# asbschmidt/CUDASW4

Hardware: AMD Instinct MI355X
Metric: GCUPS (higher is better)
Workload: dtype f16x2; 1 GPU; peak: allqueries.fasta (20 queries, 41752 residues) vs pseudo DB 1000000 x 512, half2 kernel configuration, blosum62, gop -11 gex -1, top 10, C++ host driver; db_subjects=1000000, db_residues=512000000, queries=20, kernel=half2, queries_in_flight=1, tail_overlaps=10, numa_node_rank0=1, numa_bound=True, resident=True, residency=resident, cached_chars=512000000, parallelism=db-shard x1 (one DB sharded), one top-K gather per step + host merge

## Files before the change

### cudasw4_amd/csrc/sw_api.hip

```cpp
#include <hip/hip_runtime.h>
#include <hipcub/hipcub.hpp>

#include <algorithm>
#include <cstdio>
#include <cmath>
#include <cstdlib>
#include <cstring>
#include <ctime>
#include <string>
#include <vector>

#include "../../include/cudasw4_amd.h"
#include "../../include/cudasw4_amd_engine.h"
#include "../../include/cudasw4_amd_pssm.h"
#include "sw_internal.hpp"
#include "sw_launch.hpp"
#include "sw_pssm.hpp"
#include "sw_rows_pipeline.hpp"

namespace {

thread_local std::string g_last_error = "";

int fail(int code, const std::string& msg) {
// ... 175 lines not shown
    if (part_id < SW_NUM_LENGTH_PARTITIONS - 2) {
        if (!ctx->have_query) return 16;
        const int32_t limit4 = ctx->lanes4_max_q >= 0 ? ctx->lanes4_max_q : kind_packed(kind) ? SW_LANES4_MAX_QUERY_PACKED : SW_LANES4_MAX_QUERY_SCALAR;
        const int64_t batches4 = (int64_t)n / (64 * (kind_packed(kind) ? 2 : 1));
        const bool enough4 = ctx->lanes4_max_q >= 0 || batches4 >= (int64_t)SW_LANES4_MIN_BATCHES_PER_CU * std::max(1, ctx->num_cus);
        const int32_t lmax4 = ctx->lanes4_max_subject >= 0 ? ctx->lanes4_max_subject : SW_LANES4_MAX_SUBJECT;
        if (ctx->qlen <= 4 * swk::max_rows(kind, 4) && ctx->qlen <= limit4 && enough4 && max_subject_len <= lmax4) return 4;
        const bool fits8 = ctx->qlen <= 8 * swk::max_rows(kind, 8);
        const int32_t limit = ctx->lanes8_max_q >= 0 ? ctx->lanes8_max_q : kind_packed(kind) ? SW_LANES8_MAX_QUERY_PACKED : SW_LANES8_MAX_QUERY_SCALAR;
        if (fits8 && ctx->qlen <= limit) return 8;
        return 16;
    }
    const int64_t fills_gpu_twice = (int64_t)2 * std::max(1, ctx->num_cus) * 4 * 32;
    if (part_id == SW_NUM_LENGTH_PARTITIONS - 2) return n >= (ctx->long16_min >= 0 ? ctx->long16_min : 512) ? 16 : 64;
    return n >= fills_gpu_twice ? 16 : 64;
}


int ensure_profile(sw_ctx* ctx, int kind, int lanes, int frame, int shift, hipStream_t stream) {
    Profile& pr = ctx->profiles[kind][shape_index(lanes)][frame];
    if (pr.valid && pr.shift != shift) pr.valid = false;
    if (pr.valid) {
        SW_HIP(hipStreamWaitEvent(stream, pr.ready, 0));
        return SW_OK;
    }
    const swk::KindLaunch* kl = kind_launch(kind);
    const QueryPlan pl = plan_query(kind, ctx->qlen, lanes);
    const size_t bytes = kl->tile_bytes(pl.rows, lanes) * (size_t)pl.nstripes;
    if (bytes == 0) return fail(SW_ERR_INVALID, "no kernel compiled for this query plan");
    if (bytes > pr.capacity) {
        const size_t cap = std::max<size_t>(std::max(bytes, 2 * pr.capacity), size_t(2) << 20);
        if (pr.dev) SW_HIP(hipFree(pr.dev));
        pr.dev = nullptr;
        pr.capacity = 0;
        SW_HIP(hipMalloc(&pr.dev, cap));
        pr.capacity = cap;
    }
    if (ctx->pssm_mode) SW_HIP(kl->profile(pl.rows, lanes, nullptr, ctx->qlen, ctx->d_pssm, ctx->qlen, pl.nstripes, pr.dev, shift, frame == 2 ? 1 : 0, stream));
    else SW_HIP(kl->profile(pl.rows, lanes, ctx->d_query, ctx->qlen, ctx->d_matrix, ctx->dim, pl.nstripes, pr.dev, shift, frame == 2 ? 1 : 0, stream));
    pr.shift = shift;
    if (!pr.ready) SW_HIP(hipEventCreateWithFlags(&pr.ready, hipEventDisableTiming));
    SW_HIP(hipEventRecord(pr.ready, stream));
    pr.plan = pl;
    pr.valid = true;
    return SW_OK;
}

int32_t border_capacity(int32_t max_len, int lanes) {
    const int64_t steps = ((int64_t)max_len + lanes - 1 + 3) / 4 * 4;
    return (int32_t)((steps + 15) / 16 * 16 + 16);
}
size_t border_bytes_per_wg(int32_t lcap, int lanes) {
    if (lanes == 4) return 0;
    const size_t region = lanes == 16 ? swk::border_region_words<16>(lcap) : lanes == 8 ? swk::border_region_words<8>(lcap) : swk::border_region_words<64>(lcap);
    return (size_t)(swk::kThreads / lanes) * region * sizeof(uint32_t);
}

__global__ void max_length_kernel(const int32_t* lengths, const int32_t* positions, const int32_t* count_ptr, int32_t first_pos,
                                  int32_t n, int32_t* out) {
    const int32_t cnt = count_ptr ? min(*count_ptr, n) : n;
    int32_t m = 0;
    for (int32_t i = blockIdx.x * blockDim.x + threadIdx.x; i < cnt; i += gridDim.x * blockDim.x)
        m = max(m, lengths[positions ? positions[i] : first_pos + i]);
    if (m > 0) atomicMax(out, m);
}

struct StreamPlan { int slots = 0, cols = 0, room = 0, base = 0, jump = 0; };
StreamPlan stream_plan(const sw_ctx* ctx, int kind, int lanes, int a, const QueryPlan& pl, int32_t max_subject_len) {
    StreamPlan sp;
    if (!kind_packed(kind) || lanes != 16 || a < 0) return sp;
    const bool multi = pl.nstripes > 1;
    const int P = swk::frame_classes(true, pl.rows, lanes, multi);
    sp.base = kind == SW_KIND_F16X2 ? -2016 : 0;
    const int top = kind == SW_KIND_F16X2 ? 1024 : 12400;
    sp.jump = ctx->stream_jump > 0 ? ctx->stream_jump : (kind == SW_KIND_F16X2 ? 512 : 2048);
    sp.room = top - sp.base - a * (2 * lanes + 4 + P);
    sp.cols = a > 0 ? std::min(sp.room / a, ctx->stream_cols_max) : ctx->stream_cols_max;
    sp.slots = std::max(1, std::min(ctx->stream_slots, swk::kStreamMaxSlots));
    if (sp.room < 4 * lanes * a || sp.cols < 4 * lanes) sp.slots = 1;
    if (multi) {
        const int32_t limit = ctx->stream_multi_max_subject >= 0 ? ctx->stream_multi_max_subject : (kind == SW_KIND_F16X2 ? 320 : 192);
        if (max_subject_len > limit) sp.slots = 1;
        sp.cols = std::min(sp.cols, ctx->stream_multi_cols_max);
    }
    return sp;
}

bool offs_possible(const sw_ctx* ctx, int kind, int lanes, int32_t max_subject_len, int gop, int gex, int ovf_check, int64_t* K_out) {
    const int a = -gex;
    const int64_t room = kind == SW_KIND_F16X2 ? 1536 : kind == SW_KIND_I16X2 ? 12500 : (int64_t)1 << 22;
    int64_t K = 1 << 21;
    while (K >= 4 * lanes && (int64_t)a * (K + 3 * lanes + 16) > room) K >>= 1;
    if (kind == SW_KIND_I16X2) K = std::min<int64_t>(K, std::max<int64_t>(2048, 4 * lanes));
    if (!kind_packed(kind) && max_subject_len + 3 * lanes + 16 > K) K = 0;
    if (K_out) *K_out = K;
    return ctx->use_offs && K >= 4 * lanes && (!kind_packed(kind) || (ovf_check && a >= 0)) && gop - gex >= -1000;
}
int packed_fallback_kind(int kind) { return kind == SW_KIND_F16X2 ? SW_KIND_F32 : SW_KIND_I32; }

constexpr uint32_t kWorkZeroBlock = 64;
hipError_t take_work_slot(sw_ctx* ctx, hipStream_t stream, uint32_t** out) {
    uint32_t* w = ctx->d_work + 2 * (ctx->work_next++ % kWorkSlots);
    *out = w;
    if (ctx->work_zeroed > 0) { ctx->work_zeroed--; return hipSuccess; }
    return hipMemsetAsync(w, 0, 2 * sizeof(uint32_t), stream);
}

// ... 1347 lines not shown
```

### cudasw4_amd/csrc/sw_dp_kernel.hpp

```cpp
#pragma once

#include <hip/hip_runtime.h>
#include <stdint.h>

#include <type_traits>

#include "sw_pssm.hpp"

namespace swk {

typedef uint32_t u32;
typedef short s16x2 __attribute__((ext_vector_type(2)));
typedef unsigned short u16x2 __attribute__((ext_vector_type(2)));
typedef _Float16 f16x2 __attribute__((ext_vector_type(2)));

constexpr int kGroup = 16;
constexpr int kThreads = 256;
constexpr int kPadLetter = 20;
constexpr int kLetters = 21;

enum { F16X2 = 0, I16X2 = 1, I32 = 2, F32 = 3 };

constexpr int DPP_ROW_SHL1 = 0x101;
constexpr int DPP_ROW_SHR1 = 0x111;
// ... 325 lines not shown
#define SWK_WAVES4_MAX_R 22
#endif
#ifndef SWK_CLASSES_PACKED
#define SWK_CLASSES_PACKED 8
#endif
#ifndef SWK_CLASSES_PACKED_SMALL
#define SWK_CLASSES_PACKED_SMALL 4
#endif
#ifndef SWK_CLASSES_SCALAR
#define SWK_CLASSES_SCALAR 4
#endif
constexpr int frame_classes(bool packed, int R, int lanes, bool multi, bool uniform = false) {
    (void)lanes;
    const int want = packed ? ((R > SWK_WAVES3_MAX_R || (multi && R >= 25 && (uniform || R > SWK_WAVES3_MAX_R_MULTI))) ? SWK_CLASSES_PACKED : SWK_CLASSES_PACKED_SMALL)
                            : SWK_CLASSES_SCALAR;
    int P = want;
    while (P > 1 && 2 * P > R) P--;
    return P;
}

constexpr int kLookahead = 12;

template <int NW, int CHUNK_ROW_BYTES>
__device__ __forceinline__ void lds_read_chunk2(u32 (&da)[NW], u32 (&db)[NW], const unsigned char* pa, const unsigned char* pb, int c) {
    lds_read_chunk<NW, CHUNK_ROW_BYTES>(da, pa, c);
    lds_read_chunk<NW, CHUNK_ROW_BYTES>(db, pb, c);
    __builtin_amdgcn_sched_barrier(0);
}

template <int NW, int CHUNK_ROW_BYTES>
__device__ __forceinline__ void lds_read_words2(u32 (&da)[NW], u32 (&db)[NW], const unsigned char* pa, const unsigned char* pb) {
#pragma unroll
    for (int c = 0; c < Chunks<NW>::kCount; c++) lds_read_chunk2<NW, CHUNK_ROW_BYTES>(da, db, pa, pb, c);
}

template <int NW, int CHUNK_ROW_BYTES>
__device__ __forceinline__ void lds_read_chunk1(u32 (&da)[NW], const unsigned char* pa, int c) {
    lds_read_chunk<NW, CHUNK_ROW_BYTES>(da, pa, c);
    __builtin_amdgcn_sched_barrier(0);
}

template <int KIND, int R, int P = 1>
struct StripeState {
    u32 H[R];
    u32 E[R];
    u32 upH_prev;
    u32 Hlast;
    u32 Fout;
    u32 yA, yB;
    u32 maxv[P + 3];
    u32 Zc[P + 4];
};

template <int KIND, int R, int LANES, int BYTE, bool MULTI, bool OFFS = false, int P = 1, bool ZFILL = true, bool UNI = false>
__device__ __forceinline__ void dp_step(StripeState<KIND, R, P>& st, const unsigned char* tile,
                                        u32 lettersA, u32 lettersB, u32 gop, u32 gex, u32 inH, u32 inF,
                                        u32 apos = 0, bool first = false, u32 wrapP = 0, u32 wrapLast = 0, bool head = false,
                                        u32 laneStep = 0, const u32* zw = nullptr) {
    using A = Arith<KIND>;
    using G = Geometry<KIND, R, LANES>;
    const u32 step2 = LANES < 16 ? laneStep : 0x00100010u;
    const u32 step1 = LANES < 16 ? laneStep : 16u;
    constexpr u32 kSel = 0x0c0c000cu | ((u32)BYTE << 8);
    constexpr int kPostShift = G::kLetterShift - 8;

    static_assert(!A::kPacked || OFFS, "packed kinds run the column-offset recurrence only");
    u32 wa[G::NW];
    u32 wb[G::NW];
    if constexpr (A::kPacked && LANES <= 16) {
        constexpr u32 kSel2 = ((u32)(4 + BYTE) << 24) | 0x000c000cu | ((u32)BYTE << 8);
        const u32 inj = __builtin_amdgcn_perm(lettersB, lettersA, kSel2);
        st.yA = prev_lane<LANES, false>(inj, st.yA, head) + step2;
    } else {
        const u32 injA = __builtin_amdgcn_perm(0u, lettersA, kSel) << kPostShift;
        st.yA = prev_lane<LANES, false>(injA, st.yA, head) + step1;
        if constexpr (A::kPacked || !OFFS) lds_read_words<G::NW, G::kChunkRowBytes>(wa, tile + st.yA);
        if constexpr (A::kPacked) {
            const u32 injB = __builtin_amdgcn_perm(0u, lettersB, kSel) << kPostShift;
            st.yB = prev_lane<LANES, false>(injB, st.yB, head) + step1;
            lds_read_words<G::NW, G::kChunkRowBytes>(wb, tile + st.yB);
        }
    }

    if constexpr (OFFS) {
        constexpr int kLastClass = (R - 1) % P;
        constexpr int Q = A::kWindow ? BYTE : 0;
        u32 upH, F;
        if constexpr (MULTI) {
            (void)first;
            upH = prev_lane<LANES, false>(inH, st.Hlast, head);
            F = prev_lane<LANES, false>(inF, st.Fout, head);
        } else {
            const u32 bH = UNI ? zw[Q + kLastClass] : st.Zc[Q + kLastClass];
            upH = prev_lane<LANES, false>(bH, st.Hlast, head);
            if constexpr (ZFILL) F = prev_lane<LANES, true>(0u, st.Fout, head);
            else F = prev_lane<LANES, false>(st.Zc[Q], st.Fout, head);
        }
        u32 diag = st.upH_prev;
        st.upH_prev = upH;
        u32 m[P];
#pragma unroll
        for (int c = 0; c < P; c++) m[c] = A::kWindow ? st.maxv[Q + c] : A::add(st.maxv[c], apos);
        auto score = [&](int r) -> u32 {
            if constexpr (G::kWide) return 0u;
            else if constexpr (A::kPacked) return __builtin_amdgcn_perm(wb[r >> 1], wa[r >> 1], (r & 1) ? 0x07060302u : 0x05040100u);
            else return wa[r];
        };
        auto diag_term = [&](int, u32 d, u32 sc) -> u32 { return A::add(d, sc); };
        constexpr int kAhead = G::kWide ? (kLookahead < R ? kLookahead : R) : 1;
        using CH = Chunks<G::NW>;
        constexpr int kChunksAll = CH::kCount;
        constexpr int kChunks0 = G::kWide ? CH::lead_for(kAhead, 4) : 1;
        static_assert(!G::kWide || kChunks0 >= kChunksAll || CH::lead_ok(kChunks0, kAhead, 4), "a score word would be used before its read is issued");
        const unsigned char* const pa = tile + (st.yA & 0xffffu);
        const unsigned char* const pb = tile + (st.yA >> 16);
        u32 tq[G::kWide ? R : 1];
        if constexpr (G::kWide) {
#pragma unroll
            for (int k = 0; k < kChunks0 && k < kChunksAll; k++) lds_read_chunk2<G::NW, G::kChunkRowBytes>(wa, wb, pa, pb, k);
#pragma unroll
            for (int r = 0; r < kAhead; r++) tq[r] = A::add_pair(wa[r], wb[r], r == 0 ? diag : st.H[r - 1]);
        }
        constexpr bool kProg1 = !A::kPacked;
        constexpr int kChunks0S = kProg1 ? CH::lead_for(2, 6) : 1;
        if constexpr (kProg1) {
#pragma unroll
            for (int k = 0; k < kChunks0S && k < kChunksAll; k++) lds_read_chunk1<G::NW, G::kChunkRowBytes>(wa, tile + st.yA, k);
        }
        u32 s_next = score(0);
        u32 t_next = G::kWide ? 0u : diag_term(0, diag, s_next);
        s_next = R > 1 ? score(1) : 0u;
#pragma unroll
        for (int r = 0; r < R; r++) {
            const int c = r % P;
            const u32 zop = UNI ? zw[Q + c + 2] : st.Zc[Q + c + 1];
            if constexpr (G::kWide) {
                if (r % 4 == 0) __builtin_amdgcn_sched_barrier(0);
                if (CH::starts_chunk(r) && CH::chunk_of(r) + kChunks0 < kChunksAll)
                    lds_read_chunk2<G::NW, G::kChunkRowBytes>(wa, wb, pa, pb, CH::chunk_of(r) + kChunks0);
                t_next = tq[r];
            }
            if constexpr (kProg1) {
                if (r % 4 == 0) __builtin_amdgcn_sched_barrier(0);
                if (CH::starts_chunk(r) && CH::chunk_of(r) + kChunks0S < kChunksAll)
                    lds_read_chunk1<G::NW, G::kChunkRowBytes>(wa, tile + st.yA, CH::chunk_of(r) + kChunks0S);
            }
            const u32 t = t_next;
            const u32 h = A::cell_h(t, st.E[r], F);
            const u32 s1 = s_next;
            if (r + 2 < R) s_next = score(r + 2);
            const u32 hg = A::gap(h, gop);
            if constexpr (G::kWide) {
                if (r + kAhead < R) tq[r + kAhead] = A::add_pair(wa[r + kAhead], wb[r + kAhead], st.H[r + kAhead - 1]);
            } else {
                if (r + 1 < R) t_next = diag_term(r + 1, st.H[r], s1);
            }
            const u32 fm = A::max3(F, hg, zop);
            st.E[r] = A::max3(st.E[r], hg, zop);
            if (r == R - 1) F = (UNI && kLastClass == 0) ? fm : A::gap(fm, wrapLast);
            else if (c == P - 1) F = A::gap(fm, wrapP);
            else F = fm;
            if ((r / P) & 1) m[c] = A::fold2(m[c], st.H[r - P], h);
            else if (r + P >= R) m[c] = A::max2(m[c], h);
            st.H[r] = h;
        }
#pragma unroll
        for (int c = 0; c < P; c++) st.maxv[Q + c] = m[c];
        if constexpr (!A::kWindow) {
// ... 43 lines not shown

template <class MAX>
__device__ __forceinline__ u32 half_row_max(u32 v, MAX&& mx) {
    v = mx(v, dpp<0x141, false>(v, v));
    v = mx(v, dpp<0xB1, false>(v, v));
    v = mx(v, dpp<0x4E, false>(v, v));
    return v;
}

template <class MAX>
__device__ __forceinline__ u32 quad_max(u32 v, MAX&& mx) {
    v = mx(v, dpp<0xB1, false>(v, v));
    v = mx(v, dpp<0x4E, false>(v, v));
    return v;
}

template <int KIND>
__device__ __forceinline__ u32 row_max_true(u32 v) {
    using A = Arith<KIND>;
    v = A::true_max(v, dpp<0x128, false>(v, v));
    v = A::true_max(v, dpp<0x124, false>(v, v));
    v = A::true_max(v, dpp<0x122, false>(v, v));
    v = A::true_max(v, dpp<0x121, false>(v, v));
    return v;
}

template <int KIND, int LANES>
__device__ __forceinline__ u32 group_max(u32 v) {
    using A = Arith<KIND>;
    if constexpr (LANES == 8) return half_row_max(v, [](u32 a, u32 b) { return A::max2(a, b); });
    if constexpr (LANES == 4) return quad_max(v, [](u32 a, u32 b) { return A::max2(a, b); });
    v = row_max_true<KIND>(v);
    if constexpr (LANES == 64) {
        v = A::max2(v, (u32)__shfl_xor((int)v, 16));
        v = A::max2(v, (u32)__shfl_xor((int)v, 32));
    }
    return v;
}

template <int LANES>
struct Border {
    static constexpr int kBlockCols = 2 * LANES;
    static constexpr int kQuadsPerBlock = LANES / 2;
    static constexpr int kBlockBytes = 8 * kBlockCols;
    static constexpr int kBlockWords = 2 * kBlockCols;
    static constexpr int kInBytes = kBlockBytes, kOutBytes = kBlockBytes, kDummyBytes = 8 * (kThreads / LANES) + 32;
    static constexpr int kGroupBytes = kInBytes + kOutBytes + 16;
    static constexpr int ring_bytes(int groups) { return groups * kGroupBytes + kDummyBytes; }
    static_assert(kGroupBytes % 16 == 0, "rings are read and written 16 bytes at a time");
    static constexpr int blocks(int steps) { return (steps + kBlockCols - 1) / kBlockCols + 3; }
};
template <int LANES>
constexpr int border_region_words(int lcap) { return Border<LANES>::blocks(lcap) * Border<LANES>::kBlockWords; }

__device__ __forceinline__ void announce_start(const ScanParams& p) {
    if (p.start_signal && threadIdx.x == 0) {
        if (atomicAdd(p.work_counter + 1, 1u) + 1u == p.start_quorum)
            __hip_atomic_fetch_add(p.start_signal, 1u, __ATOMIC_RELEASE, __HIP_MEMORY_SCOPE_SYSTEM);
    }
}

#ifndef SWK_I32_WAVES3_MAX_R
#define SWK_I32_WAVES3_MAX_R 32
#endif
#ifndef SWK_I32_WAVES3_MAX_R_MULTI
#define SWK_I32_WAVES3_MAX_R_MULTI 32
#endif
#ifndef SWK_F32_WAVES3_MAX_R
#define SWK_F32_WAVES3_MAX_R 48
#endif
#ifndef SWK_F32_WAVES3_MAX_R_MULTI
#define SWK_F32_WAVES3_MAX_R_MULTI 48
#endif
constexpr int min_waves_of(int KIND, int R, int LANES, bool MULTI) {
    const bool packed = KIND == F16X2 || KIND == I16X2;
    if (packed && LANES <= 16 && MULTI && R <= SWK_WAVES3_MAX_R_MULTI) return 3;
    if (packed) return (LANES <= 16 && !MULTI && R <= SWK_WAVES4_MAX_R) ? 4 : (LANES <= 16 && !MULTI && R <= SWK_WAVES3_MAX_R) ? 3 : 2;
    if (KIND == I32 && LANES <= 16 && R > (MULTI ? SWK_I32_WAVES3_MAX_R_MULTI : SWK_I32_WAVES3_MAX_R)) return 2;
    if (KIND == F32 && LANES <= 16 && R > (MULTI ? SWK_F32_WAVES3_MAX_R_MULTI : SWK_F32_WAVES3_MAX_R)) return 2;
    return (R <= 16 && !MULTI && LANES <= 16) ? 4 : 3;
}
template <int KIND, int R, int LANES, bool MULTI>
constexpr int min_waves() { return min_waves_of(KIND, R, LANES, MULTI); }
constexpr int vgpr_slot_of(int KIND, int R, int LANES, bool MULTI) { return (512 / min_waves_of(KIND, R, LANES, MULTI)) & ~7; }

template <int KIND, int R, int LANES, bool MULTI, bool OFFS = false>
__global__ void __launch_bounds__(kThreads, (min_waves<KIND, R, LANES, MULTI>())) sw_scan_kernel(const ScanParams p) {
    using A = Arith<KIND>;
    using G = Geometry<KIND, R, LANES>;
    constexpr int kGroups = kThreads / LANES;
    using BD = Border<LANES>;
    constexpr int SHL1 = Shift<LANES>::kShl1;
    constexpr int kQuadsPerLetterBlock = LANES;
    static_assert(!A::kPacked || OFFS, "packed kinds run the column-offset recurrence only (sw_launch.hpp: launch_scan_ro)");
    constexpr bool kUni = A::kPacked;
    constexpr int P = OFFS ? frame_classes(A::kPacked, R, LANES, MULTI, kUni) : 1;
    __shared__ __attribute__((aligned(16))) unsigned char lds[16 + G::kTileBytes];
    __shared__ __attribute__((aligned(16))) unsigned char rings[MULTI ? BD::ring_bytes(kGroups) : 16];

    const int tid = threadIdx.x;
    const int lane = tid & (LANES - 1);
    const int group = tid / LANES;
    const bool head = lane == 0;
    const int slot = LANES < 16 ? (tid & 15) : lane;
    const u32 laneStep = (A::kPacked ? 0x00100010u : 16u) * ((LANES < 16 && head) ? u32(slot + 1) : 1u);
    announce_start(p);
    if (p.positions) __builtin_amdgcn_s_setprio(2);
    const bool service = p.service != 0;
    const int n = (p.count_ptr && !service) ? *p.count_ptr : p.n;
    constexpr int kSubjPerBatch = kGroups * A::kSubjects;
    const int nbatches = (n + kSubjPerBatch - 1) / kSubjPerBatch;
    if (!service && (int)blockIdx.x >= nbatches) return;

    if constexpr (!MULTI) {
        load_tile<G::kTileBytes>(lds, p.profile);
        __syncthreads();
    }

    unsigned char* const ringIn = rings + (MULTI ? group * BD::kGroupBytes : 0);
    unsigned char* const ringOut = ringIn + BD::kInBytes;
    u32* const gBorder = MULTI ? p.scratch + ((size_t)blockIdx.x * kGroups + group) * (size_t)border_region_words<LANES>(p.lcap) : nullptr;

    const u32 apos = OFFS ? A::pos_word(p.gex_mag) : 0u;
    const u32 apos4 = OFFS ? A::pos_word(4 * p.gex_mag) : 0u;
    const int rq = kUni ? p.renorm_quads : 0;
    const int kmask = 4 * rq - 1;
    const u32 zstart = (OFFS && !kUni) ? A::zero_at(p.gex_mag, LANES - lane) : A::kZero;
    const u32 zbefore = (OFFS && !kUni) ? A::zero_at(p.gex_mag, LANES - lane - 1) : A::kZero;

    __shared__ int next_batch, batch_avail;
    auto claim_entry = [&](int i) -> int {
        for (int spin = 0; spin < (1 << 20); spin++) {
            const int v = __hip_atomic_load(p.claim + i, __ATOMIC_RELAXED, __HIP_MEMORY_SCOPE_AGENT);
            if (v == kListTaken) return -1;
            if (v >= 0) return atomicCAS(p.claim + i, v, kListTaken) == v ? v : -1;
            __builtin_amdgcn_s_sleep(2);
        }
        return -1;
    };
    for (;;) {
        __syncthreads();
        if (tid == 0) {
            int b = (int)atomicAdd(p.work_counter, 1u), avail = n;
            if (service) {
                avail = 0;
                for (u32 spin = 0; b < nbatches; spin++) {
                    avail = __hip_atomic_load(p.count_ptr, __ATOMIC_RELAXED, __HIP_MEMORY_SCOPE_AGENT);
                    if (avail > b * kSubjPerBatch) break;
                    const u32 done = __hip_atomic_load(p.done_flag, __ATOMIC_RELAXED, __HIP_MEMORY_SCOPE_SYSTEM);
                    if ((int32_t)(done - p.done_value) >= 0 || spin > 600000u) { b = nbatches; break; }
                    __builtin_amdgcn_s_sleep(127);
                }
                avail = min(avail, n);
            }
            if (b == nbatches && p.dry_signal) __hip_atomic_store(p.dry_signal, p.dry_value, __ATOMIC_RELAXED, __HIP_MEMORY_SCOPE_SYSTEM);
            next_batch = b;
            batch_avail = avail;
        }
        __syncthreads();
        const int b = next_batch;
        if (b >= nbatches) break;
        const int navail = batch_avail;
        const int batch = service ? b : nbatches - 1 - b;
        const int i0 = batch * kSubjPerBatch + group * A::kSubjects;
        const int i1 = i0 + 1;
        bool valid0 = i0 < navail;
        bool valid1 = A::kPacked && (i1 < navail);
        int pos0 = 0, pos1 = 0, len0 = 0, len1 = 0;
        const int8_t* s0 = p.chars;
        const int8_t* s1 = p.chars;
        if (p.claim) {
            int v = -1;
            if (valid0 && lane == 0) v = claim_entry(i0);
            if constexpr (LANES == 64) v = __builtin_amdgcn_readfirstlane(v);
            else v = __shfl(v, (tid & 63) & ~(LANES - 1));
            valid0 = v >= 0;
            pos0 = valid0 ? v : 0;
            if (valid0) {
                len0 = p.lengths[pos0];
                s0 = p.chars + (p.offsets[pos0] - p.offsets[0]);
            }
            valid1 = false;
        } else {
            if (valid0) {
                pos0 = p.positions ? p.positions[i0] : p.first_pos + i0;
                len0 = p.lengths[pos0];
                s0 = p.chars + (p.offsets[pos0] - p.offsets[0]);
            }
            if (valid1) {
                pos1 = p.positions ? p.positions[i1] : p.first_pos + i1;
                len1 = p.lengths[pos1];
                s1 = p.chars + (p.offsets[pos1] - p.offsets[0]);
            }
        }
        int lmax = len0 > len1 ? len0 : len1;
        if constexpr (LANES <= 16) {
            if constexpr (LANES <= 4) lmax = max(lmax, __shfl_xor(lmax, 4));
            if constexpr (LANES <= 8) lmax = max(lmax, __shfl_xor(lmax, 8));
            lmax = max(lmax, __shfl_xor(lmax, 16));
            lmax = max(lmax, __shfl_xor(lmax, 32));
        }
        int nquads = (lmax + LANES - 1 + 3) >> 2;
        if constexpr (MULTI) nquads = min(nquads, (p.lcap - 4) >> 2);
        nquads = __builtin_amdgcn_readfirstlane(nquads);
        const int len0pad = (len0 + 3) & ~3, len1pad = (len1 + 3) & ~3;

        u32 maxv = 0u;
        for (int stripe = 0; stripe < p.nstripes; stripe++) {
            const bool first = stripe == 0;
            if constexpr (MULTI) {
                __syncthreads();
                load_tile<G::kTileBytes>(lds, p.profile + (size_t)stripe * G::kTileBytes);
                __syncthreads();
            }
            StripeState<KIND, R, P> st;
            u32 zw[P + 5];
            const int tg0 = kUni ? __builtin_amdgcn_readfirstlane(LANES * stripe) : 0;
            auto load_levels = [&](int q) {
                const int u0 = __builtin_amdgcn_readfirstlane((tg0 + 4 * q) & kmask);
#pragma unroll
                for (int k = 0; k < P + 5; k++) zw[k] = p.levels[u0 + k];
#pragma unroll
                for (int k = 0; k < P + 5; k++) asm volatile("" : "+s"(zw[k]));
            };
            if constexpr (kUni) {
                load_levels(0);
#pragma unroll
                for (int r = 0; r < R; r++) { st.H[r] = zw[r % P]; st.E[r] = zw[r % P + 1]; }
                st.upH_prev = A::gap(zw[(R - 1) % P], p.gex); st.Hlast = zw[(R - 1) % P]; st.Fout = zw[0];
#pragma unroll
                for (int d = 0; d < P + 3; d++) st.maxv[d] = A::add(maxv, zw[d + 1]);
            } else {
                u32 zc[P + 5];
                zc[0] = zbefore; zc[1] = zstart;
#pragma unroll
                for (int k = 2; k < P + 5; k++) zc[k] = A::add(zc[k - 1], apos);
#pragma unroll
                for (int r = 0; r < R; r++) { st.H[r] = zc[r % P]; st.E[r] = zc[r % P + 1]; }
                st.upH_prev = zc[(R - 1) % P]; st.Hlast = zc[(R - 1) % P]; st.Fout = zbefore;
#pragma unroll
                for (int k = 0; k < P + 4; k++) st.Zc[k] = zc[k + 1];
#pragma unroll
                for (int d = 0; d < P + 3; d++) st.maxv[d] = OFFS ? A::add(maxv, zc[A::kWindow ? d + 1 : d]) : maxv;
            }
            st.yA = ((u32)(kPadLetter * G::kLetterUnits) << G::kLetterShift) + 16u * (u32)(slot + 1);
            st.yB = st.yA;
            if constexpr (A::kPacked && LANES <= 16) st.yA |= st.yA << 16;

            auto fetch = [&](const int8_t* s, int lenpad, int blk) -> u32 {
                const int j = blk * (4 * LANES) + lane * 4;
                u32 w = 0x14141414u;
                if (j < lenpad) w = *reinterpret_cast<const u32*>(s + j);
                return w * (u32)G::kLetterUnits;
            };
            u32 nextA = fetch(s0, len0pad, 0);
            u32 nextB = A::kPacked ? fetch(s1, len1pad, 0) : 0u;
            u32 lettersA = 0, lettersB = 0;

            const bool last = stripe + 1 == p.nstripes;
            const unsigned char* inPtr = ringIn;
            unsigned char* outPtr = (lane == LANES - 1) ? ringOut : rings + kGroups * BD::kGroupBytes + 8 * group;
            const u32 walkIn = 32u;
            const u32 walkOut = (lane == LANES - 1) ? 32u : 0u;
            uint4 pend = make_uint4(A::kZero, A::kZero, A::kZero, A::kZero);
            uint2 nxt = make_uint2(A::kZero, A::kZero);
            const u32* const gIn = MULTI ? gBorder + 2 * (LANES - 1) + 4 * lane : nullptr;
            auto first_stripe_pairs = [&](int j) -> uint4 {
                if constexpr (kUni) {
                    constexpr int kLastClass = (R - 1) % P;
                    return make_uint4(A::zero_at(p.gex_mag, (j & kmask) + kLastClass), A::kZero, A::zero_at(p.gex_mag, ((j + 1) & kmask) + kLastClass), A::kZero);
                } else if constexpr (OFFS) {
                    constexpr int kLastClass = (R - 1) % P;
                    const int K = 4 * rq;
                    const int j0 = K > 0 ? (j & (K - 1)) : j, j1 = K > 0 ? ((j + 1) & (K - 1)) : j + 1;
                    return make_uint4(A::zero_at(p.gex_mag, j0 + LANES + kLastClass), A::kZero, A::zero_at(p.gex_mag, j1 + LANES + kLastClass), A::kZero);
                } else {
                    return make_uint4(A::kZero, A::kZero, A::kZero, A::kZero);
                }
            };
            if constexpr (MULTI) {
                __builtin_amdgcn_fence(__ATOMIC_ACQUIRE, "workgroup");
                if (!first) {
                    const uint4 b0 = *reinterpret_cast<const uint4*>(gIn);
                    pend = *reinterpret_cast<const uint4*>(gIn + BD::kBlockWords);
                    *reinterpret_cast<uint4*>(ringIn + 16 * lane) = b0;
                } else {
                    *reinterpret_cast<uint4*>(ringIn + 16 * lane) = first_stripe_pairs(2 * lane);
                }
                __builtin_amdgcn_fence(__ATOMIC_RELEASE, "wavefront");
                nxt = *reinterpret_cast<const uint2*>(inPtr);
            }
            auto block_end = [&](int blk) {
                int t = tid;
                asm volatile("" : "+v"(t));
                const int ln = t & (LANES - 1), grp = t / LANES;
                unsigned char* const rIn = rings + grp * BD::kGroupBytes + 16 * ln;
                u32* const gb = p.scratch + ((size_t)blockIdx.x * kGroups + grp) * (size_t)border_region_words<LANES>(p.lcap) + 4 * ln;
                __builtin_amdgcn_fence(__ATOMIC_ACQ_REL, "wavefront");
                if (!last) {
                    const uint4 v = *reinterpret_cast<const uint4*>(rIn + BD::kInBytes);
                    *reinterpret_cast<uint4*>(gb + (size_t)blk * BD::kBlockWords) = v;
                }
                outPtr -= walkOut * BD::kQuadsPerBlock;
                inPtr -= walkIn * BD::kQuadsPerBlock;
                if (first) {
                    *reinterpret_cast<uint4*>(rIn) = first_stripe_pairs((blk + 1) * BD::kBlockCols + 2 * ln);
                } else {
                    *reinterpret_cast<uint4*>(rIn) = pend;
                    pend = *reinterpret_cast<const uint4*>(gb + 2 * (LANES - 1) + (size_t)(blk + 2) * BD::kBlockWords);
                }
                __builtin_amdgcn_fence(__ATOMIC_ACQ_REL, "wavefront");
                nxt = *reinterpret_cast<const uint2*>(inPtr);
            };

            auto lower_frame = [&]() {
                if constexpr (kUni) {
                    const u32 w = p.renorm_word;
#pragma unroll
                    for (int r = 0; r < R; r++) { st.H[r] = A::lower(st.H[r], w); st.E[r] = A::lower(st.E[r], w); }
                    st.upH_prev = A::lower(st.upH_prev, w);
                    if constexpr (KIND == I16X2) st.upH_prev = A::true_max(st.upH_prev, A::gap(A::kZero, p.gex));
                    st.Hlast = A::lower(st.Hlast, w);
                    st.Fout = A::lower(st.Fout, w);
#pragma unroll
                    for (int d = 0; d < P + 3; d++) st.maxv[d] = A::lower(st.maxv[d], w);
                }
            };
            auto quad = [&](int q) {
                if ((q & (kQuadsPerLetterBlock - 1)) == 0) {
                    lettersA = nextA; lettersB = nextB;
                    nextA = fetch(s0, len0pad, q / kQuadsPerLetterBlock + 1);
                    if constexpr (A::kPacked) nextB = fetch(s1, len1pad, q / kQuadsPerLetterBlock + 1);
                }
                const bool lower = kUni && ((tg0 + 4 * q + 4) & kmask) == 0;
                auto border_step = [&](auto byte_tag) {
                    constexpr int BYTE = decltype(byte_tag)::value;
                    const uint2 in = nxt;
                    if constexpr (MULTI) {
                        if constexpr (BYTE == 3) {
                            inPtr += walkIn;
                            nxt = *reinterpret_cast<const uint2*>(inPtr);
                        } else {
                            nxt = *reinterpret_cast<const uint2*>(inPtr + 8 * (BYTE + 1));
                        }
                    }
                    dp_step<KIND, R, LANES, BYTE, MULTI, OFFS, P, true, kUni>(st, lds, lettersA, lettersB, p.gop, p.gex, in.x, in.y, apos, first,
                                                                          p.wrap_class, p.wrap_last, head, laneStep, zw);
                    if constexpr (kUni && BYTE == 3) {
                        if (lower) lower_frame();
                    }
                    if constexpr (MULTI) *reinterpret_cast<uint2*>(outPtr + 8 * BYTE) = make_uint2(st.Hlast, st.Fout);
                };
                border_step(std::integral_constant<int, 0>{});
                border_step(std::integral_constant<int, 1>{});
                border_step(std::integral_constant<int, 2>{});
                border_step(std::integral_constant<int, 3>{});
                if constexpr (MULTI) outPtr += walkOut;
                lettersA = dpp<SHL1, true>(0u, lettersA);
                if constexpr (A::kPacked) lettersB = dpp<SHL1, true>(0u, lettersB);
                if constexpr (OFFS && A::kWindow) {
                    if constexpr (!kUni) {
#pragma unroll
                        for (int k = 0; k < P + 4; k++) st.Zc[k] = A::add(st.Zc[k], apos4);
                    }
#pragma unroll
                    for (int d = 0; d < P + 3; d++) st.maxv[d] = A::add(st.maxv[d], apos4);
                }
                if constexpr (kUni) load_levels(q + 1);
            };
            if constexpr (!MULTI) {
                for (int q = 0; q < nquads; q++) quad(q);
            } else {
                for (int q0 = 0; q0 < nquads; q0 += BD::kQuadsPerBlock) {
                    const int qend = min(nquads, q0 + BD::kQuadsPerBlock);
                    for (int q = q0; q < qend; q++) quad(q);
                    if (qend == q0 + BD::kQuadsPerBlock) block_end(q0 / BD::kQuadsPerBlock);
                }
            }
            if constexpr (MULTI) {
                if (!last) {
                    const int done = nquads & ~(BD::kQuadsPerBlock - 1);
                    const int slot = 4 * (nquads - done) + lane;
                    u32* const g = gBorder + (size_t)(done / BD::kQuadsPerBlock) * BD::kBlockWords;
                    __builtin_amdgcn_fence(__ATOMIC_ACQ_REL, "wavefront");
                    if (slot < BD::kBlockCols) *reinterpret_cast<uint2*>(ringOut + 8 * slot) = make_uint2(A::kZero, A::kZero);
                    else *reinterpret_cast<uint2*>(g + 2 * slot) = make_uint2(A::kZero, A::kZero);
                    __builtin_amdgcn_fence(__ATOMIC_ACQ_REL, "wavefront");
                    *reinterpret_cast<uint4*>(g + 4 * lane) = *reinterpret_cast<const uint4*>(ringOut + 16 * lane);
                }
            }
            if constexpr (kUni) {
                maxv = A::true_of(st.maxv[0], zw[1]);
#pragma unroll
                for (int d = 1; d < P + 3; d++) maxv = A::true_max(maxv, A::true_of(st.maxv[d], zw[d + 1]));
            } else if constexpr (OFFS) {
                if constexpr (A::kWindow) {
                    maxv = A::true_of(st.maxv[0], st.Zc[0]);
#pragma unroll
                    for (int d = 1; d < P + 3; d++) maxv = A::true_max(maxv, A::true_of(st.maxv[d], st.Zc[d]));
                } else {
                    maxv = A::true_of(st.maxv[0], A::gap(A::gap(st.Zc[1], p.gex), p.gex));
#pragma unroll
                    for (int c = 1; c < P; c++)
                        maxv = A::true_max(maxv, A::true_of(st.maxv[c], A::gap(A::gap(st.Zc[c + 1], p.gex), p.gex)));
                }
            } else {
                maxv = st.maxv[0];
            }
            if constexpr (MULTI) __builtin_amdgcn_fence(__ATOMIC_RELEASE, "workgroup");
        }

        int sc0, sc1, guard = 0;
// ... 88 lines not shown
```

### cudasw4_amd/csrc/sw_stream_kernel.hpp

```cpp
#pragma once
#include "sw_dp_kernel.hpp"

namespace swk {

constexpr int kStreamMaxSlots = 16;

template <int KIND, int R, int LANES, bool MULTI>
__global__ void __launch_bounds__(kThreads, (min_waves<KIND, R, LANES, MULTI>())) sw_scan_stream_kernel(const ScanParams p) {
    using A = Arith<KIND>;
    using G = Geometry<KIND, R, LANES>;
    static_assert(A::kPacked && A::kWindow && LANES == 16, "streamed subjects: the packed windowed kernels on 16-lane groups");
    static_assert(kStreamMaxSlots <= LANES, "lane k of a group keeps slot k's running maximum");
    constexpr int kGroups = kThreads / LANES;
    constexpr int kWaves = kThreads / 64;
    using BD = Border<LANES>;
    constexpr int SHL1 = Shift<LANES>::kShl1;
    constexpr int kQuadsPerLetterBlock = LANES;
    constexpr int P = frame_classes(true, R, LANES, MULTI);
    constexpr int kLastClass = (R - 1) % P;
    constexpr int kSubjPerBatch = kGroups * 2;
    constexpr int kMinWidth = 2 * LANES;
    __shared__ __attribute__((aligned(16))) unsigned char lds[16 + G::kTileBytes];
    __shared__ __attribute__((aligned(16))) unsigned char rings[MULTI ? BD::ring_bytes(kGroups) : 16];
    __shared__ int slotBnd[kWaves][kStreamMaxSlots + 1];
    __shared__ int next_batch, claimed;

    const int tid = threadIdx.x;
    const int lane = tid & (LANES - 1);
    const int group = tid / LANES;
    const int wave = tid >> 6;
    const bool head = lane == 0;
    const u32 laneStep = 0x00100010u;
    announce_start(p);
    const int n = p.n;
    const int nbatches = (n + kSubjPerBatch - 1) / kSubjPerBatch;
    if ((int)blockIdx.x >= nbatches) return;
    if constexpr (!MULTI) load_tile<G::kTileBytes>(lds, p.profile);

    unsigned char* const ringIn = rings + (MULTI ? group * BD::kGroupBytes : 0);
    unsigned char* const ringOut = ringIn + BD::kInBytes;
    u32* const gBorder = MULTI ? p.scratch + ((size_t)blockIdx.x * kGroups + group) * (size_t)border_region_words<LANES>(p.lcap) : nullptr;

    const int a = p.gex_mag;
    const u32 apos = A::pos_word(a);
    const u32 apos4 = A::pos_word(4 * a);
    const u32 zstart = A::level_word(p.level_base + a * (LANES - lane));
    const u32 zbefore = A::level_word(p.level_base + a * (LANES - lane - 1));
    const int smax = min(max(p.stream_slots, 1), kStreamMaxSlots);

    for (;;) {
        __syncthreads();
        if (tid < 64) {
            int cur = 0;
            if (tid == 0) cur = (int)__hip_atomic_load(p.work_counter, __ATOMIC_RELAXED, __HIP_MEMORY_SCOPE_AGENT);
            cur = __shfl(cur, 0);
            const int want = max(1, min(smax, (nbatches - cur) / (int)gridDim.x));
            const int k = tid;
            const int batch = nbatches - 1 - (cur + k);
            const bool in = k < want && batch >= 0;
            int w = 0;
            if (in) w = max(p.lengths[p.first_pos + min(n - 1, batch * kSubjPerBatch + kSubjPerBatch - 1)] + (k > 0 ? 1 : 0), kMinWidth);
            int c = w;
#pragma unroll
            for (int d = 1; d < LANES; d <<= 1) {
                const int u = __shfl_up(c, d, LANES);
                if ((k & (LANES - 1)) >= d) c += u;
            }
            const bool ok = in && (k == 0 || (c <= p.stream_cols && a * c + k * p.jump <= p.stream_room));
            const unsigned long long m = __ballot(ok) & ((1ull << kStreamMaxSlots) - 1ull);
            const int take = max(1, __ffsll((long long)~m) - 1);
            if (tid == 0) {
                const int b = (int)atomicAdd(p.work_counter, (u32)take);
                if (b <= nbatches && b + take > nbatches && p.dry_signal)
                    __hip_atomic_store(p.dry_signal, p.dry_value, __ATOMIC_RELAXED, __HIP_MEMORY_SCOPE_SYSTEM);
                next_batch = b;
                claimed = take;
            }
        }
        __syncthreads();
        const int b0 = __builtin_amdgcn_readfirstlane(next_batch);
        if (b0 >= nbatches) break;
        const int S = __builtin_amdgcn_readfirstlane(min(claimed, nbatches - b0));

        u32 soff0 = 0, soff1 = 0;
        u32 slens = 0;
        {
            int slen0 = 0, slen1 = 0;
            if (lane < S) {
                const int batch = nbatches - 1 - (b0 + lane);
                const int i0 = batch * kSubjPerBatch + group * 2;
                if (i0 < n) { slen0 = p.lengths[p.first_pos + i0]; soff0 = (u32)((p.offsets[p.first_pos + i0] - p.offsets[0]) >> 2); }
                if (i0 + 1 < n) { slen1 = p.lengths[p.first_pos + i0 + 1]; soff1 = (u32)((p.offsets[p.first_pos + i0 + 1] - p.offsets[0]) >> 2); }
            }
            slens = (u32)slen0 | ((u32)slen1 << 16);
// ... 75 lines not shown
                zc[0] = zbefore; zc[1] = zstart;
#pragma unroll
                for (int k = 2; k < P + 5; k++) zc[k] = A::add(zc[k - 1], apos);
#pragma unroll
                for (int r = 0; r < R; r++) { st.H[r] = zc[r % P]; st.E[r] = zc[r % P + 1]; }
                st.upH_prev = zc[(R - 1) % P]; st.Hlast = zc[(R - 1) % P]; st.Fout = zbefore;
#pragma unroll
                for (int k = 0; k < P + 4; k++) st.Zc[k] = zc[k + 1];
#pragma unroll
                for (int d = 0; d < P + 3; d++) st.maxv[d] = zc[d + 1];
            }
            st.yA = ((u32)(kPadLetter * G::kLetterUnits) << G::kLetterShift) + 16u * (u32)(lane + 1);
            st.yB = st.yA;
            st.yA |= st.yA << 16;

            u32 nextA, nextB, lettersA = 0, lettersB = 0;
            fetch2(0, nextA, nextB);
            u32 stashv = 0u;

            const unsigned char* inPtr = ringIn;
            unsigned char* outPtr = (lane == LANES - 1) ? ringOut : rings + kGroups * BD::kGroupBytes + 8 * group;
            const u32 walkIn = 32u;
            const u32 walkOut = (lane == LANES - 1) ? 32u : 0u;
            uint4 pend = make_uint4(0u, 0u, 0u, 0u);
            uint2 nxt = make_uint2(0u, 0u);
            const u32* const gIn = MULTI ? gBorder + 2 * (LANES - 1) + 4 * lane : nullptr;
            auto level_of = [&](int j) -> int {
                const int K = 4 * rq;
                int lv = p.level_base + a * ((K > 0 ? (j & (K - 1)) : j) + LANES);
                for (int i = 1; i < S; i++) lv += (j >= slotBnd[wave][i]) ? p.jump : 0;
                return lv;
            };
            auto first_stripe_pairs = [&](int j) -> uint4 {
                const int l0 = level_of(j), l1 = level_of(j + 1);
                return make_uint4(A::level_word(l0 + a * kLastClass), A::level_word(l0), A::level_word(l1 + a * kLastClass), A::level_word(l1));
            };
            if constexpr (MULTI) {
                __builtin_amdgcn_fence(__ATOMIC_ACQUIRE, "workgroup");
                if (!first) {
                    const uint4 b0w = *reinterpret_cast<const uint4*>(gIn);
                    pend = *reinterpret_cast<const uint4*>(gIn + BD::kBlockWords);
                    *reinterpret_cast<uint4*>(ringIn + 16 * lane) = b0w;
                } else {
                    *reinterpret_cast<uint4*>(ringIn + 16 * lane) = first_stripe_pairs(2 * lane);
                }
                __builtin_amdgcn_fence(__ATOMIC_RELEASE, "wavefront");
                nxt = *reinterpret_cast<const uint2*>(inPtr);
            }
            auto block_end = [&](int blk) {
                int t = tid;
                asm volatile("" : "+v"(t));
                const int ln = t & (LANES - 1), grp = t / LANES;
                unsigned char* const rIn = rings + grp * BD::kGroupBytes + 16 * ln;
                u32* const gb = p.scratch + ((size_t)blockIdx.x * kGroups + grp) * (size_t)border_region_words<LANES>(p.lcap) + 4 * ln;
                __builtin_amdgcn_fence(__ATOMIC_ACQ_REL, "wavefront");
                if (!last) {
                    const uint4 v = *reinterpret_cast<const uint4*>(rIn + BD::kInBytes);
                    *reinterpret_cast<uint4*>(gb + (size_t)blk * BD::kBlockWords) = v;
                }
                outPtr -= walkOut * BD::kQuadsPerBlock;
                inPtr -= walkIn * BD::kQuadsPerBlock;
                if (first) {
                    *reinterpret_cast<uint4*>(rIn) = first_stripe_pairs((blk + 1) * BD::kBlockCols + 2 * ln);
                } else {
                    *reinterpret_cast<uint4*>(rIn) = pend;
                    pend = *reinterpret_cast<const uint4*>(gb + 2 * (LANES - 1) + (size_t)(blk + 2) * BD::kBlockWords);
                }
                __builtin_amdgcn_fence(__ATOMIC_ACQ_REL, "wavefront");
                nxt = *reinterpret_cast<const uint2*>(inPtr);
            };

            int ksl = 1;
            int evb = S > 1 ? __builtin_amdgcn_readfirstlane(slotBnd[wave][1]) : (rq > 0 ? 4 * rq : 0x3fffffff);
            int evq0 = evb >> 2, evq1 = (evb + LANES - 1) >> 2;

            auto switch_lane = [&](int ksw) {
                u32 m = A::true_of(st.maxv[0], st.Zc[0]);
#pragma unroll
                for (int d = 1; d + 1 < P + 3; d += 2)
                    m = A::fold2(m, A::true_of(st.maxv[d], st.Zc[d]), A::true_of(st.maxv[d + 1], st.Zc[d + 1]));
                if constexpr ((P + 3) % 2 == 0) m = A::true_max(m, A::true_of(st.maxv[P + 2], st.Zc[P + 2]));
                const bool me = lane == ksw;
                stashv = me ? m : stashv;
                const u32 gw = me ? p.jump_word : 0u;
#pragma unroll
                for (int i = 0; i < P + 4; i++) st.Zc[i] = A::add(st.Zc[i], gw);
            };
            auto quad = [&](int q, auto mode_tag) {
                constexpr int MODE = decltype(mode_tag)::value;
                if ((q & (kQuadsPerLetterBlock - 1)) == 0) {
                    lettersA = nextA; lettersB = nextB;
                    fetch2(q / kQuadsPerLetterBlock + 1, nextA, nextB);
                }
                const int lower_lane = 4 * (q & (rq - 1));
                auto lower_frame = [&](int k) {
                    const u32 gw = lane == k ? p.renorm_word : 0u;
#pragma unroll
                    for (int r = 0; r < R; r++) { st.H[r] = A::gap(st.H[r], gw); st.E[r] = A::gap(st.E[r], gw); }
                    st.upH_prev = A::gap(st.upH_prev, gw);
#pragma unroll
                    for (int k2 = 0; k2 < P + 4; k2++) st.Zc[k2] = A::gap(st.Zc[k2], gw);
#pragma unroll
                    for (int d = 0; d < P + 3; d++) st.maxv[d] = A::gap(st.maxv[d], gw);
                };
                auto border_step = [&](auto byte_tag) {
                    constexpr int BYTE = decltype(byte_tag)::value;
                    if constexpr (MODE == 2) switch_lane(4 * q + BYTE - evb);
// ... 120 lines not shown
```

Before: 11920 GCUPS.

## Precompute per-subject profile address stream in global scratch for packed multi-stripe kernel

For the packed 16-lane multi-stripe scan, the kernel now writes, once per subject pair, an interleaved stream of scaled letter offsets for both subjects into an extra scratch region appended to each group's border area. During the DP, each lane reads its column addresses from this stream instead of fetching letters per block, injecting them through lane shifts and doing DPP shifts of the letter registers. This aims to cut per-step VALU and cross-lane work in the inner loop. The cost is a larger scratch footprint, an extra global write pass per subject, and an extra global load every few steps.

```diff
diff --git a/cudasw4_amd/csrc/sw_api.hip b/cudasw4_amd/csrc/sw_api.hip
--- a/cudasw4_amd/csrc/sw_api.hip
+++ b/cudasw4_amd/csrc/sw_api.hip
@@ -251,7 +251,7 @@
 }
 size_t border_bytes_per_wg(int32_t lcap, int lanes) {
     if (lanes == 4) return 0;
-    const size_t region = lanes == 16 ? swk::border_region_words<16>(lcap) : lanes == 8 ? swk::border_region_words<8>(lcap) : swk::border_region_words<64>(lcap);
+    const size_t region = lanes == 16 ? swk::group_region_words<16>(lcap) : lanes == 8 ? swk::group_region_words<8>(lcap) : swk::group_region_words<64>(lcap);
     return (size_t)(swk::kThreads / lanes) * region * sizeof(uint32_t);
 }
 
diff --git a/cudasw4_amd/csrc/sw_dp_kernel.hpp b/cudasw4_amd/csrc/sw_dp_kernel.hpp
--- a/cudasw4_amd/csrc/sw_dp_kernel.hpp
+++ b/cudasw4_amd/csrc/sw_dp_kernel.hpp
@@ -401,7 +401,7 @@
     u32 Zc[P + 4];
 };
 
-template <int KIND, int R, int LANES, int BYTE, bool MULTI, bool OFFS = false, int P = 1, bool ZFILL = true, bool UNI = false>
+template <int KIND, int R, int LANES, int BYTE, bool MULTI, bool OFFS = false, int P = 1, bool ZFILL = true, bool UNI = false, bool ADDR = false>
 __device__ __forceinline__ void dp_step(StripeState<KIND, R, P>& st, const unsigned char* tile,
                                         u32 lettersA, u32 lettersB, u32 gop, u32 gex, u32 inH, u32 inF,
                                         u32 apos = 0, bool first = false, u32 wrapP = 0, u32 wrapLast = 0, bool head = false,
@@ -416,7 +416,9 @@
     static_assert(!A::kPacked || OFFS, "packed kinds run the column-offset recurrence only");
     u32 wa[G::NW];
     u32 wb[G::NW];
-    if constexpr (A::kPacked && LANES <= 16) {
+    static_assert(!ADDR || (A::kPacked && LANES == 16 && OFFS), "the address stream serves the packed kinds on 16-lane groups");
+    if constexpr (ADDR) {
+    } else if constexpr (A::kPacked && LANES <= 16) {
         constexpr u32 kSel2 = ((u32)(4 + BYTE) << 24) | 0x000c000cu | ((u32)BYTE << 8);
         const u32 inj = __builtin_amdgcn_perm(lettersB, lettersA, kSel2);
         st.yA = prev_lane<LANES, false>(inj, st.yA, head) + step2;
@@ -461,8 +463,8 @@
         constexpr int kChunksAll = CH::kCount;
         constexpr int kChunks0 = G::kWide ? CH::lead_for(kAhead, 4) : 1;
         static_assert(!G::kWide || kChunks0 >= kChunksAll || CH::lead_ok(kChunks0, kAhead, 4), "a score word would be used before its read is issued");
-        const unsigned char* const pa = tile + (st.yA & 0xffffu);
-        const unsigned char* const pb = tile + (st.yA >> 16);
+        const unsigned char* const pa = ADDR ? tile + 16 + __builtin_amdgcn_perm(lettersA, laneStep, 0x0c0c0500u) : tile + (st.yA & 0xffffu);
+        const unsigned char* const pb = ADDR ? tile + 16 + __builtin_amdgcn_perm(lettersA, laneStep, 0x0c0c0700u) : tile + (st.yA >> 16);
         u32 tq[G::kWide ? R : 1];
         if constexpr (G::kWide) {
 #pragma unroll
@@ -612,6 +614,11 @@
 };
 template <int LANES>
 constexpr int border_region_words(int lcap) { return Border<LANES>::blocks(lcap) * Border<LANES>::kBlockWords; }
+
+template <int LANES>
+constexpr int stream_region_words(int lcap) { return LANES == 16 ? Border<LANES>::blocks(lcap) * Border<LANES>::kBlockCols : 0; }
+template <int LANES>
+constexpr int group_region_words(int lcap) { return border_region_words<LANES>(lcap) + stream_region_words<LANES>(lcap); }
 
 __device__ __forceinline__ void announce_start(const ScanParams& p) {
     if (p.start_signal && threadIdx.x == 0) {
@@ -654,6 +661,7 @@
     constexpr int kQuadsPerLetterBlock = LANES;
     static_assert(!A::kPacked || OFFS, "packed kinds run the column-offset recurrence only (sw_launch.hpp: launch_scan_ro)");
     constexpr bool kUni = A::kPacked;
+    constexpr bool kAddr = A::kPacked && MULTI && LANES == 16;
     constexpr int P = OFFS ? frame_classes(A::kPacked, R, LANES, MULTI, kUni) : 1;
     __shared__ __attribute__((aligned(16))) unsigned char lds[16 + G::kTileBytes];
     __shared__ __attribute__((aligned(16))) unsigned char rings[MULTI ? BD::ring_bytes(kGroups) : 16];
@@ -663,7 +671,7 @@
     const int group = tid / LANES;
     const bool head = lane == 0;
     const int slot = LANES < 16 ? (tid & 15) : lane;
-    const u32 laneStep = (A::kPacked ? 0x00100010u : 16u) * ((LANES < 16 && head) ? u32(slot + 1) : 1u);
+    const u32 laneStep = kAddr ? 16u * (u32)slot : (A::kPacked ? 0x00100010u : 16u) * ((LANES < 16 && head) ? u32(slot + 1) : 1u);
     announce_start(p);
     if (p.positions) __builtin_amdgcn_s_setprio(2);
     const bool service = p.service != 0;
@@ -679,7 +687,19 @@
 
     unsigned char* const ringIn = rings + (MULTI ? group * BD::kGroupBytes : 0);
     unsigned char* const ringOut = ringIn + BD::kInBytes;
-    u32* const gBorder = MULTI ? p.scratch + ((size_t)blockIdx.x * kGroups + group) * (size_t)border_region_words<LANES>(p.lcap) : nullptr;
+    u32* const gBorder = MULTI ? p.scratch + ((size_t)blockIdx.x * kGroups + group) * (size_t)group_region_words<LANES>(p.lcap) : nullptr;
+    typedef const __attribute__((address_space(1))) unsigned char* StreamPtr;
+    StreamPtr streamBase = nullptr;
+    u32 streamOff = 0;
+    if constexpr (kAddr) {
+        constexpr int kGroupsPerWave = 64 / LANES;
+        const int g0 = group & ~(kGroupsPerWave - 1);
+        const uintptr_t b = reinterpret_cast<uintptr_t>(p.scratch + ((size_t)blockIdx.x * kGroups + g0) * (size_t)group_region_words<LANES>(p.lcap) +
+                                                        border_region_words<LANES>(p.lcap));
+        streamBase = (StreamPtr)(((uintptr_t)(u32)__builtin_amdgcn_readfirstlane((int)(b >> 32)) << 32) |
+                                 (uintptr_t)(u32)__builtin_amdgcn_readfirstlane((int)(u32)b));
+        streamOff = 4u * (u32)((group - g0) * group_region_words<LANES>(p.lcap) + LANES - lane);
+    }
 
     const u32 apos = OFFS ? A::pos_word(p.gex_mag) : 0u;
     const u32 apos4 = OFFS ? A::pos_word(4 * p.gex_mag) : 0u;
@@ -764,6 +784,21 @@
         if constexpr (MULTI) nquads = min(nquads, (p.lcap - 4) >> 2);
         nquads = __builtin_amdgcn_readfirstlane(nquads);
         const int len0pad = (len0 + 3) & ~3, len1pad = (len1 + 3) & ~3;
+        auto letters4 = [&](const int8_t* s, int lenpad, int j) -> u32 {
+            u32 w = 0x14141414u;
+            if (j < lenpad) w = *reinterpret_cast<const u32*>(s + j);
+            return w * (u32)G::kLetterUnits;
+        };
+        if constexpr (kAddr) {
+            u32* const sw = gBorder + border_region_words<LANES>(p.lcap) + LANES;
+            sw[lane - LANES] = (u32)(kPadLetter * G::kLetterUnits) * 0x01000100u;
+            for (int c = lane; c < nquads + LANES / 4; c += LANES) {
+                const u32 a = letters4(s0, len0pad, 4 * c), b = letters4(s1, len1pad, 4 * c);
+                *reinterpret_cast<uint4*>(sw + 4 * c) = make_uint4(__builtin_amdgcn_perm(b, a, 0x040c000cu), __builtin_amdgcn_perm(b, a, 0x050c010cu),
+                                                                   __builtin_amdgcn_perm(b, a, 0x060c020cu), __builtin_amdgcn_perm(b, a, 0x070c030cu));
+            }
+            __builtin_amdgcn_fence(__ATOMIC_RELEASE, "workgroup");
+        }
 
         u32 maxv = 0u;
         for (int stripe = 0; stripe < p.nstripes; stripe++) {
@@ -808,14 +843,15 @@
             if constexpr (A::kPacked && LANES <= 16) st.yA |= st.yA << 16;
 
             auto fetch = [&](const int8_t* s, int lenpad, int blk) -> u32 {
-                const int j = blk * (4 * LANES) + lane * 4;
-                u32 w = 0x14141414u;
-                if (j < lenpad) w = *reinterpret_cast<const u32*>(s + j);
-                return w * (u32)G::kLetterUnits;
+                if constexpr (kAddr) return 0u;
+                else return letters4(s, lenpad, blk * (4 * LANES) + lane * 4);
             };
             u32 nextA = fetch(s0, len0pad, 0);
             u32 nextB = A::kPacked ? fetch(s1, len1pad, 0) : 0u;
             u32 lettersA = 0, lettersB = 0;
+            StreamPtr streamAt = streamBase;
+            auto stream_word = [&](int k) -> u32 { return ((const __attribute__((address_space(1))) u32*)(streamAt + (size_t)streamOff))[k]; };
+            u32 nxtW = 0;
 
             const bool last = stripe + 1 == p.nstripes;
             const unsigned char* inPtr = ringIn;
@@ -849,13 +885,14 @@
                 }
                 __builtin_amdgcn_fence(__ATOMIC_RELEASE, "wavefront");
                 nxt = *reinterpret_cast<const uint2*>(inPtr);
+                if constexpr (kAddr) nxtW = stream_word(0);
             }
             auto block_end = [&](int blk) {
                 int t = tid;
                 asm volatile("" : "+v"(t));
                 const int ln = t & (LANES - 1), grp = t / LANES;
                 unsigned char* const rIn = rings + grp * BD::kGroupBytes + 16 * ln;
-                u32* const gb = p.scratch + ((size_t)blockIdx.x * kGroups + grp) * (size_t)border_region_words<LANES>(p.lcap) + 4 * ln;
+                u32* const gb = p.scratch + ((size_t)blockIdx.x * kGroups + grp) * (size_t)group_region_words<LANES>(p.lcap) + 4 * ln;
                 __builtin_amdgcn_fence(__ATOMIC_ACQ_REL, "wavefront");
                 if (!last) {
                     const uint4 v = *reinterpret_cast<const uint4*>(rIn + BD::kInBytes);
@@ -887,7 +924,7 @@
                 }
             };
             auto quad = [&](int q) {
-                if ((q & (kQuadsPerLetterBlock - 1)) == 0) {
+                if (!kAddr && (q & (kQuadsPerLetterBlock - 1)) == 0) {
                     lettersA = nextA; lettersB = nextB;
                     nextA = fetch(s0, len0pad, q / kQuadsPerLetterBlock + 1);
                     if constexpr (A::kPacked) nextB = fetch(s1, len1pad, q / kQuadsPerLetterBlock + 1);
@@ -904,8 +941,17 @@
                             nxt = *reinterpret_cast<const uint2*>(inPtr + 8 * (BYTE + 1));
                         }
                     }
-                    dp_step<KIND, R, LANES, BYTE, MULTI, OFFS, P, true, kUni>(st, lds, lettersA, lettersB, p.gop, p.gex, in.x, in.y, apos, first,
-                                                                          p.wrap_class, p.wrap_last, head, laneStep, zw);
+                    if constexpr (kAddr) {
+                        lettersA = nxtW;
+                        if constexpr (BYTE == 3) {
+                            streamAt += 16;
+                            nxtW = stream_word(0);
+                        } else {
+                            nxtW = stream_word(BYTE + 1);
+                        }
+                    }
+                    dp_step<KIND, R, LANES, BYTE, MULTI, OFFS, P, true, kUni, kAddr>(st, lds, lettersA, lettersB, p.gop, p.gex, in.x, in.y, apos, first,
+                                                                                 p.wrap_class, p.wrap_last, head, laneStep, zw);
                     if constexpr (kUni && BYTE == 3) {
                         if (lower) lower_frame();
                     }
@@ -916,8 +962,10 @@
                 border_step(std::integral_constant<int, 2>{});
                 border_step(std::integral_constant<int, 3>{});
                 if constexpr (MULTI) outPtr += walkOut;
-                lettersA = dpp<SHL1, true>(0u, lettersA);
-                if constexpr (A::kPacked) lettersB = dpp<SHL1, true>(0u, lettersB);
+                if constexpr (!kAddr) {
+                    lettersA = dpp<SHL1, true>(0u, lettersA);
+                    if constexpr (A::kPacked) lettersB = dpp<SHL1, true>(0u, lettersB);
+                }
                 if constexpr (OFFS && A::kWindow) {
                     if constexpr (!kUni) {
 #pragma unroll
diff --git a/cudasw4_amd/csrc/sw_stream_kernel.hpp b/cudasw4_amd/csrc/sw_stream_kernel.hpp
--- a/cudasw4_amd/csrc/sw_stream_kernel.hpp
+++ b/cudasw4_amd/csrc/sw_stream_kernel.hpp
@@ -39,7 +39,7 @@
 
     unsigned char* const ringIn = rings + (MULTI ? group * BD::kGroupBytes : 0);
     unsigned char* const ringOut = ringIn + BD::kInBytes;
-    u32* const gBorder = MULTI ? p.scratch + ((size_t)blockIdx.x * kGroups + group) * (size_t)border_region_words<LANES>(p.lcap) : nullptr;
+    u32* const gBorder = MULTI ? p.scratch + ((size_t)blockIdx.x * kGroups + group) * (size_t)group_region_words<LANES>(p.lcap) : nullptr;
 
     const int a = p.gex_mag;
     const u32 apos = A::pos_word(a);
@@ -221,7 +221,7 @@
                 asm volatile("" : "+v"(t));
                 const int ln = t & (LANES - 1), grp = t / LANES;
                 unsigned char* const rIn = rings + grp * BD::kGroupBytes + 16 * ln;
-                u32* const gb = p.scratch + ((size_t)blockIdx.x * kGroups + grp) * (size_t)border_region_words<LANES>(p.lcap) + 4 * ln;
+                u32* const gb = p.scratch + ((size_t)blockIdx.x * kGroups + grp) * (size_t)group_region_words<LANES>(p.lcap) + 4 * ln;
                 __builtin_amdgcn_fence(__ATOMIC_ACQ_REL, "wavefront");
                 if (!last) {
                     const uint4 v = *reinterpret_cast<const uint4*>(rIn + BD::kInBytes);
```

After: 12090 GCUPS (median of 6 runs). 1.01x the previous value.
